# hjmkt/wrenc

Measured on AMD Instinct MI355X. Metric: all-intra encode fps at fixed QP (CTU RD search + final pass); bit-exactness vs the CPU oracle is checked in `parity`, higher is better.
Workload: dtype u8/i16/i32 (+i64 trellis costs, f32 RD cost)

## Files before the change

wrenc_amd/csrc/dev_common.h:

```cpp
#pragma once
#include <cstddef>
#include <type_traits>

namespace wrenc {

enum { PLANAR = 0, DC = 1, LT_CCLM = 81, L_CCLM = 82, T_CCLM = 83 };
enum { TREE_SINGLE = 0, TREE_DUAL_LUMA = 1, TREE_DUAL_CHROMA = 2 };

struct DevConst {
    int32_t W, H, qp, max_depth, ctu_cols, ctu_rows;
    int32_t lsc;
    uint32_t div_magic;
    uint32_t div_shift;
    int64_t lambda_q;
    float lambda_rd;
    float lambda_rd_chroma;
    int64_t ldq[1024];
    int64_t lv[1024];
    int64_t hb_luma[2][4][67];
    int64_t hb_chroma[4];
    int16_t dct[4][32][32];
    int16_t dct_t[4][32][32];
    uint8_t diag4[16][2];
    uint8_t diag_sb[4][64][2];
// ... 129 lines not shown
    UF<float> cur_cost;
    uint32_t pad3_;
    UF<float> cost;
    EvalPartsU e_best;
};

template <class T>
struct SF {
    T v;
    UF<T>* p;
    __device__ __forceinline__ T get() const { return v; }
    __device__ __forceinline__ operator T() const { return v; }
    __device__ __forceinline__ SF& operator=(T x) {
        v = x;
        p->set(x);
        return *this;
    }
    __device__ __forceinline__ SF& operator=(const SF& o) { return *this = o.v; }
    __device__ __forceinline__ SF& operator+=(int x) { return *this = (T)(v + x); }
    __device__ __forceinline__ SF& operator-=(int x) { return *this = (T)(v - x); }
};
struct EvalPartsSF {
    SF<uint32_t> ssd_y, ssd_c;
    SF<long long> lvl_y, lvl_c;
    __device__ __forceinline__ EvalParts get() const {
        EvalParts e;
        e.ssd_y = ssd_y;
        e.ssd_c = ssd_c;
        e.lvl_y = lvl_y;
        e.lvl_c = lvl_c;
        return e;
    }
};
struct LeafSF {
    SF<uint8_t> cont, op_ml, op_mc, op_act, bx, by, lg, need_refs0, need_refs1, need_org, cur_mode, mode,
        cclm_mode, holder, evalr, luma_mode, chroma_mode, best_cls, need_save, tile_best, slot;
    SF<float> best_cost, cur_cost, cost;
    EvalPartsSF e_best;
};
static_assert(sizeof(LeafSt) == 64, "snap_leaf reads the struct as 16 dwords");
__device__ __forceinline__ LeafSF snap_leaf(LeafSt& l) {
    __builtin_amdgcn_fence(__ATOMIC_ACQ_REL, "wavefront");
    const int w = ((const int*)&l)[LANE & 15];
    LeafSF s;
#define SNAP_U8(f)                                                                                          \
    s.f.v = (uint8_t)((unsigned)__builtin_amdgcn_readlane(w, (int)(offsetof(LeafSt, f) >> 2)) >> (8 * (offsetof(LeafSt, f) & 3))); \
    s.f.p = &l.f
#define SNAP_F32(f)                                                                       \
    s.f.v = __int_as_float(__builtin_amdgcn_readlane(w, (int)(offsetof(LeafSt, f) >> 2))); \
    s.f.p = &l.f
    SNAP_U8(cont); SNAP_U8(op_ml); SNAP_U8(op_mc); SNAP_U8(op_act); SNAP_U8(bx); SNAP_U8(by); SNAP_U8(lg);
    SNAP_U8(need_refs0); SNAP_U8(need_refs1); SNAP_U8(need_org); SNAP_U8(cur_mode); SNAP_U8(mode);
    SNAP_U8(cclm_mode); SNAP_U8(holder); SNAP_U8(evalr); SNAP_U8(luma_mode); SNAP_U8(chroma_mode);
    SNAP_U8(best_cls); SNAP_U8(need_save); SNAP_U8(tile_best); SNAP_U8(slot);
    SNAP_F32(best_cost); SNAP_F32(cur_cost); SNAP_F32(cost);
#undef SNAP_U8
#undef SNAP_F32
    constexpr int eb = (int)(offsetof(LeafSt, e_best) >> 2);
    s.e_best.ssd_y.v = (uint32_t)__builtin_amdgcn_readlane(w, eb + (int)(offsetof(EvalPartsU, ssd_y) >> 2));
    s.e_best.ssd_y.p = &l.e_best.ssd_y;
    s.e_best.ssd_c.v = (uint32_t)__builtin_amdgcn_readlane(w, eb + (int)(offsetof(EvalPartsU, ssd_c) >> 2));
    s.e_best.ssd_c.p = &l.e_best.ssd_c;
    {
        constexpr int o = eb + (int)(offsetof(EvalPartsU, lvl_y) >> 2);
        s.e_best.lvl_y.v = (long long)(((unsigned long long)(unsigned)__builtin_amdgcn_readlane(w, o + 1) << 32) |
                                       (unsigned)__builtin_amdgcn_readlane(w, o));
        s.e_best.lvl_y.p = &l.e_best.lvl_y;
    }
    {
        constexpr int o = eb + (int)(offsetof(EvalPartsU, lvl_c) >> 2);
        s.e_best.lvl_c.v = (long long)(((unsigned long long)(unsigned)__builtin_amdgcn_readlane(w, o + 1) << 32) |
                                       (unsigned)__builtin_amdgcn_readlane(w, o));
        s.e_best.lvl_c.p = &l.e_best.lvl_c;
    }
    return s;
}

struct CtuSt {
    UF<uint8_t> cont, in_leaf, xpar;
    UF<uint8_t> level, bx, by, lg, max_depth;
    uint8_t pad0_;
    UF<uint8_t> z, rl, rc;
    UF<uint8_t> rbx, rby, rlg;
    UF<uint8_t> ns_luma_cur, ns_chroma_cur;
    UF<uint8_t> pend, pbx, pby, plg, pslot;
    UF<uint8_t> dp0, dp1;
    UF<uint8_t> lvmode, lv_i, zend;
    UF<uint8_t> fz_on;
    UF<float> ret, ns_cost_cur;
    uint32_t pad1_;
    UF<float> ctu_cost;
    UF<float> lv_acc0, lv_acc1;
    LeafSt leaf;
};

struct XRes {
    uint32_t ssd_y, ssd_c;
    long long lvl_y, lvl_c;
};

constexpr int R_L0 = 0, R_A0 = 66, R_LF = 130, R_AF = 196, R_LC0 = 260, R_LC1 = 294, R_AC0 = 328, R_AC1 = 360;

typedef uint8_t ref_t;
struct __attribute__((aligned(16))) Lds {
    int16_t r1[1024];
    int32_t r2[512];
    ref_t refs[392];
    uint8_t recYtop[72];
    uint8_t recY[32 * 36];
    uint8_t recCtop[2][40];
    uint8_t recC[2][16 * 20];
    uint32_t decw[128];
    int32_t slot_xfer;
    uint32_t fsum;
    uint16_t q_pm[3][4][4];
    uint8_t cu_log2[64];
    uint8_t luma_mode[64];
    uint8_t chroma_mode[16];
    uint8_t left_mode[8];
    union {
        float ns_cost[4];
        uint32_t lev_was[4];
    };
    union {
        float split_cost[4];
        uint32_t lev_now[4];
    };
    uint8_t ns_luma[4], ns_chroma[4], child[4];
    CtuSt st;
    XRes xr[2];
};

struct Ctx {
    const CONST_AS DevConst* k;
    const GLOBAL_AS uint8_t* org;
    int W, WH;
    uint8_t* pred_scratch;
    GLOBAL_AS uint8_t* slots;
    unsigned long long* mismatch;
    int ctu_x, ctu_y;
    int cu32_mode;
    int write;
    int member;
    int store;
    int solo;
    int trace;
};

#ifndef WRENC_WPB
#define WRENC_WPB 4
#endif
constexpr int WPB = WRENC_WPB;
constexpr int kWorkgroupsPerCU = 20 / WPB;
constexpr int kTeam = 4;
struct LvBox {
    float ns_cost[3], split[3];
    uint8_t ml[3], mc[3];
    uint16_t pad_;
    uint32_t cnt[3][2];
    uint32_t srv_ready, job_posted, job_done, job_ack, job_fin;
    uint32_t job4_posted, job4_done, job4_ack, job4_fin;
    uint8_t job_bx, job_by, job4_bx, job4_by;
};
struct LdsTab {
    int32_t ldq[256];
    int32_t lv[256];
    int8_t fc[32][4];
    LvBox lvb;
#ifdef WRENC_EXP_LDS_PAD
    char pad[WRENC_EXP_LDS_PAD];
#endif
};
// ... 201 lines not shown
```

wrenc_amd/csrc/dev_search.h:

```cpp
#pragma once

namespace wrenc {

enum { K_SADLIST = 0, K_FULL = 1, K_NOP = 2, K_SADSEARCH = 3, K_CCLMSEARCH = 4, K_SERVE8 = 5, K_LEAF8 = 7, K_LEAF16 = 8, K_SPLIT8 = 9, K_SERVE4 = 10 };
enum { COPY_NONE = 0, COPY_SAVE = 1, COPY_RESTORE = 2, COPY_PULL = 3 };

#if defined(WRENC_TRACE) || defined(WRENC_EXHAUSTIVE_SPLITS)
constexpr bool kSplitCut = false;
#else
constexpr bool kSplitCut = true;
#endif

#if defined(WRENC_TRACE) || defined(WRENC_EXHAUSTIVE_CANDIDATES)
constexpr bool kCandidateCut = false;
#else
constexpr bool kCandidateCut = true;
#endif

struct Req {
    int kind;
    int comps;
    int tx, ty, tlg;
    int ml, mc;
    bool active;
    bool refs0, refs1;
    bool final;
    int stage;
    int copy_from;
    bool xchg;
    int tree;
    int pre_copy, copy_comps, copy_slot, copy_tx, copy_ty, copy_tlg;
    float fcur;
};

struct Res {
    uint32_t ssd_y, ssd_c;
    long long lvl_y, lvl_c;
    float v0;
    float vmin;
    int imin;
    int imin2;
};
__device__ __forceinline__ Res res_none() {
    Res r;
    r.ssd_y = 0;
    r.ssd_c = 0;
    r.lvl_y = 0;
    r.lvl_c = 0;
    r.v0 = r.vmin = 3.40282347e+38f;
    r.imin = 0;
    r.imin2 = 0;
    return r;
}

__device__ __forceinline__ float uni_f(float v) { return __int_as_float(uni(__float_as_int(v))); }

__device__ __forceinline__ unsigned checksum_weight(int i) { return (2u * (unsigned)i + 1u) * 0x9E3779B1u; }
__device__ __forceinline__ unsigned tile_checksum(int comp, int cx, int cy, int lg) {
    const int n = 1 << lg, nn = n * n, nb = comp ? 2 : 1;
    unsigned h = 0;
    for (int i = LANE; i < nb * nn; i += 64) {
        const int blk = i >> (2 * lg), ii = i & (nn - 1);
        h += (unsigned)rec_get(comp + blk, cx + (ii & (n - 1)), cy + (ii >> lg)) * checksum_weight(i);
    }
    return (unsigned)wave_sum_i32((int)h);
}

__device__ __forceinline__ void full_front(const Ctx& c, const Req& q, int comp, int mode, int rbase,
                                           CclmPick pick = CclmPick{}) {
    const int cs = comp ? 1 : 0;
    const int nb = comp ? 2 : 1;
    const int lg = q.tlg - cs;
    PROF_MARK(tr0_);
    if ((comp ? q.refs1 : q.refs0) && mode < LT_CCLM) build_refs(c, comp, q.tx, q.ty, q.tlg);
    if (q.final) {
        const unsigned h = tile_checksum(comp, q.tx >> cs, q.ty >> cs, lg);
        if (LANE == 0) SH.fsum = h;
        WSYNC();
    }
    PROF_MARK(t0_);
    PROF_ADD2(PH_REFS, tr0_, t0_);
    predict<true>(c, comp, q.tx, q.ty, q.tlg, mode, rbase, PRED_TILE, 0, pick);
    PROF_MARK(t1_);
    PROF_ADD2(PH_PREDICT, t0_, t1_);
    fwd_dct_lg(c, lg, nb, rbase);
    PROF_MARK(t2_);
    PROF_ADD2(PH_FDCT, t1_, t2_);
// ... 137 lines not shown
        int e0 = kNoMode, e1 = kNoMode, e2 = kNoMode, e3 = kNoMode, e4 = kNoMode, e5 = kNoMode;
        const int st = r == 1 ? 2 : 1;
        if (r == 0) {
            n = 13;
            lo = 2ULL | (7ULL << 8) | (13ULL << 16) | (18ULL << 24) | (23ULL << 32) | (29ULL << 40) | (34ULL << 48) | (39ULL << 56);
            hi = 45ULL | (50ULL << 8) | (55ULL << 16) | (60ULL << 24) | (66ULL << 32);
        } else if (six) {
            e0 = !(cm < 4) ? cm - 2 : kNoMode;
            e1 = !(cm + 2 > 66) ? cm + 2 : kNoMode;
            e2 = !(cm < 5) ? cm - 3 : kNoMode;
            e3 = !(cm < 3) ? cm - 1 : kNoMode;
            e4 = !(cm + 1 > 66) ? cm + 1 : kNoMode;
            e5 = !(cm + 3 > 66) ? cm + 3 : kNoMode;
            n = 6;
            lo = (unsigned long long)e0 | ((unsigned long long)e1 << 8) | ((unsigned long long)e2 << 16) | ((unsigned long long)e3 << 24) |
                 ((unsigned long long)e4 << 32) | ((unsigned long long)e5 << 40);
        } else {
            e0 = !(cm < 2 + st) ? cm - st : kNoMode;
            e1 = !(cm + st > 66) ? cm + st : kNoMode;
            n = 2;
            lo = (unsigned long long)e0 | ((unsigned long long)e1 << 8);
        }
        const unsigned acc = sad_list_angular(c, q.comps, q.tx, q.ty, q.tlg, n, lo, hi);
        const int my_mode = LANE < n ? (int)(((LANE < 8 ? lo : hi) >> (8 * (LANE & 7))) & 255u) : kNoMode;
        const unsigned s0 = (unsigned)__builtin_amdgcn_readlane((int)acc, 0), s1 = (unsigned)__builtin_amdgcn_readlane((int)acc, 1);
        bool traced = my_mode != kNoMode;
        if (r == 0) {
            const int key = my_mode != kNoMode ? (int)((acc << 4) | (unsigned)LANE) : 0x7FFFFFFF;
            const int kmin = wave_min_i32(key);
            const int j = (kmin & 15) + 2;
            cm = j < 8 ? (int)((0x3A5C90D0E08080ULL >> (7 * j)) & 127) : (int)((0x109E3764B53A2ULL >> (7 * (j - 8))) & 127);
            cur = (unsigned)kmin >> 4;
        } else if (six) {
            const unsigned s2 = (unsigned)__builtin_amdgcn_readlane((int)acc, 2), s3 = (unsigned)__builtin_amdgcn_readlane((int)acc, 3);
            const unsigned s4 = (unsigned)__builtin_amdgcn_readlane((int)acc, 4), s5 = (unsigned)__builtin_amdgcn_readlane((int)acc, 5);
            const unsigned c0 = e0 != kNoMode ? s0 : kNoSad, c1 = e1 != kNoMode ? s1 : kNoSad;
            const unsigned mn = min(min(cur, c0), c1);
            int d = 0;
            if (cur == mn) {
            } else if (c0 == mn) {
                d = -2;
                cur = c0;
            } else {
                d = 2;
                cur = c1;
            }
            const int elo = d < 0 ? e2 : (d == 0 ? e3 : e4), ehi = d < 0 ? e3 : (d == 0 ? e4 : e5);
            const unsigned slo = d < 0 ? s2 : (d == 0 ? s3 : s4), shi = d < 0 ? s3 : (d == 0 ? s4 : s5);
            const unsigned p0 = elo != kNoMode ? slo : kNoSad, p1 = ehi != kNoMode ? shi : kNoSad;
            cm += d;
            const unsigned mn2 = min(min(cur, p0), p1);
            if (cur == mn2) {
            } else if (p0 == mn2) {
                cm -= 1;
                cur = p0;
            } else {
                cm += 1;
                cur = p1;
            }
            const int ilo = d < 0 ? 2 : (d == 0 ? 3 : 4);
            traced = traced && (LANE < 2 || LANE == ilo || LANE == ilo + 1);
        } else {
            const unsigned c0 = e0 != kNoMode ? s0 : kNoSad, c1 = e1 != kNoMode ? s1 : kNoSad;
            const unsigned mn = min(min(cur, c0), c1);
            if (cur == mn) {
            } else if (c0 == mn) {
                cm -= st;
                cur = c0;
            } else {
                cm += st;
                cur = c1;
            }
        }
        if (c.trace && traced)
            TRACE_REC(c.ctu_x + q.tx, c.ctu_y + q.ty, q.tlg, q.tree, (q.comps & 1) ? 0 : 2, (q.comps & 1) ? my_mode : 0, my_mode,
                      __float_as_int((float)acc));
    }
    cm_out = cm;
    smin_out = cur;
}

__device__ __forceinline__ Res leaf8_search(const Ctx& c, const Req& q, int* overflow);
__device__ __forceinline__ Res leaf16_search(const Ctx& c, const Req& q, int* overflow);
__device__ __forceinline__ Res split8_search(const Ctx& c, const Req& q, int* overflow);
__device__ __forceinline__ void serve_pack4(const Ctx& c, const Req& q, int* overflow);
__device__ __forceinline__ void serve_pack8(const Ctx& c, const Req& q, int* overflow);

__device__ __forceinline__ int cclm_probe(const Ctx& c, int tx, int ty, int lg, int tree, CclmParams* all) {
    const int lane = lane_fresh();
    const unsigned acc = sad_list_cclm(c, tx, ty, lg, all);
    const unsigned lt = (unsigned)__builtin_amdgcn_readlane((int)acc, 0), t = (unsigned)__builtin_amdgcn_readlane((int)acc, 1),
                   l = (unsigned)__builtin_amdgcn_readlane((int)acc, 2);
    if (c.trace && lane < 3)
        TRACE_REC(c.ctu_x + tx, c.ctu_y + ty, lg, tree, 2, 0, lane == 0 ? LT_CCLM : (lane == 1 ? T_CCLM : L_CCLM),
                  __float_as_int((float)acc));
    return (lt <= t && lt <= l) ? LT_CCLM : (t <= l ? T_CCLM : L_CCLM);
}

__device__ __forceinline__ int cclm_pred4_lane(const Ctx& c, const Req& q, const CclmPick& pick, int pl, int x, int y) {
    int v = 128;
    if (!pick.flat128) {
        const int ds = cclm_ds6(c, q.tx, q.ty, 2 * y, 2 * x, pick.avail_l);
        v = (M24(ds, pl ? pick.a1 : pick.a0) >> (pl ? pick.k1 : pick.k0)) + (pl ? pick.b1 : pick.b0);
        v = min(max(v, 0), 255);
    }
    return v;
}

template <bool TEAM, bool D3>
__device__ __forceinline__ Res evaluate(const Ctx& c, const PicBufs& pb, const Req& q, int* overflow) {
    Res r = res_none();
    PROF_MARK(tcp0_);
    if (q.pre_copy != COPY_NONE)
        copy_block(c, q.pre_copy, q.copy_comps, q.copy_slot, q.copy_tx, q.copy_ty, q.copy_tlg, q.copy_from);
    PROF_MARK(tcp1_);
    PROF_ADD2(PH_COPY, tcp0_, tcp1_);
    if (q.kind == K_NOP) return r;
    if (q.stage) stage_org_leaf(c, q.stage, q.tx, q.ty, q.tlg);
    if (q.kind == K_LEAF8) return leaf8_search(c, q, overflow);
    if (q.kind == K_LEAF16) return leaf16_search(c, q, overflow);
    if (D3 && q.kind == K_SPLIT8) return split8_search(c, q, overflow);
    if (TEAM && q.kind == K_SERVE8) {
        serve_pack8(c, q, overflow);
        return r;
    }
    if (TEAM && D3 && q.kind == K_SERVE4) {
        serve_pack4(c, q, overflow);
        return r;
    }
    int mc = q.mc;
    CclmPick cpick_ = CclmPick{};
    if (q.kind == K_CCLMSEARCH) {
        if (q.tlg > 4) stage_org(c, 2, q.tx, q.ty, q.tlg);
        CclmParams call_;
        mc = cclm_probe(c, q.tx, q.ty, q.tlg, q.tree, &call_);
        r.imin = mc;
        cpick_ = cclm_pick(call_, 2 * cclm_mode_index(mc));
    }
    if (q.kind == K_FULL || q.kind == K_CCLMSEARCH) {
#pragma unroll 1
        for (int round = 0; round < 2; ++round) {
            const int cset = q.comps & (1 << round);
            if (!cset) continue;
            if (q.active) {
#pragma unroll 1
                for (int comp = 0; comp < 2; ++comp)
                    if ((cset >> comp) & 1) {
                        PROF_MARK(tf0_);
                        full_front(c, q, comp, comp ? mc : q.ml, 0, cpick_);
                        PROF_MARK(tf1_);
                        PROF_ADD2(PH_PSZ + ((q.tlg - 2) * 2 + comp), tf0_, tf1_);
                        PROF_ADD2(PH_PCNT + ((q.tlg - 2) * 2 + comp), 0, 1);
                    }
            }
            PROF_MARK(ts0_);
            bool any_y = false, any_c = false;
            {
                bool any = false;
                long long lvl = 0;
                if (q.active)
                    lvl = quantize_solo(c, q.tlg - round, round ? 2 : 1, overflow, &any);
                if (round) {
                    r.lvl_c = lvl;
                    any_c = any;
                } else {
                    r.lvl_y = lvl;
                    any_y = any;
                }
            }
            PROF_MARK(ts1_);
            PROF_ADD2(PH_QZ + ((q.tlg - 2) & 3), ts0_, ts1_);
            if (!q.active) {
                PROF_ADD2(PH_SKIP, ts0_, ts1_);
                continue;
            }
#pragma unroll 1
            for (int comp = 0; comp < 2; ++comp) {
                if (!((cset >> comp) & 1)) continue;
                PROF_MARK(tb0_);
                const uint32_t ssd = full_back(c, pb, q, comp, 0, comp ? any_c : any_y);
                PROF_MARK(tb1_);
                PROF_ADD2(PH_PSZ + ((q.tlg - 2) * 2 + comp), tb0_, tb1_);
                if (comp)
                    r.ssd_c = ssd;
                else
                    r.ssd_y = ssd;
            }
        }
        return r;
    }
    PROF_MARK(tr0_);
    if (q.refs0 && (q.comps & 1)) build_refs(c, 0, q.tx, q.ty, q.tlg);
    if (q.refs1 && (q.comps & 2)) build_refs(c, 1, q.tx, q.ty, q.tlg);
    if (q.tlg > 4) stage_org(c, q.comps, q.tx, q.ty, q.tlg);
    PROF_MARK(t0_);
    PROF_ADD2(PH_REFS, tr0_, t0_);
    if (q.kind == K_SADSEARCH) {
        constexpr unsigned kNoSad = 0xFFFFFFFFu;
        int cm;
        unsigned smin = kNoSad;
        sad_search(c, q, cm, smin);
        r.imin = uni(cm);
        r.vmin = smin == kNoSad ? 3.40282347e+38f : uni_f((float)smin);
    } else {
// ... 767 lines not shown
}

__device__ __forceinline__ Res leaf16_search(const Ctx& c, const Req& q, int* overflow) {
    Res r = res_none();
    const int lane = lane_fresh();
    if (q.refs0) build_refs(c, 0, q.tx, q.ty, 4);
    if (q.refs1) build_refs(c, 1, q.tx, q.ty, 4);
    LeafBest best = leaf_best_init(PLANAR);
    const MpmList mpl_ = mpm_list(c, q.tx, q.ty, 4);
    {
        PROF_MARK(la0_);
        const Pack16Out a = pack16_eval(c, q, 2, PLANAR, DC, overflow);
        leaf_candidate(c, q.tx, q.ty, 4, TREE_SINGLE, mpl_, best, 0, PLANAR, pack_parts(a, 0));
        leaf_candidate(c, q.tx, q.ty, 4, TREE_SINGLE, mpl_, best, 1, DC, pack_parts(a, 1));
        pack16_to_tile(c, q, 2, best.win);
        PROF_MARK(la1_);
        PROF_ADD2(PH_LEAF + 4, la0_, la1_);
    }
    int cm;
    unsigned smin;
    PROF_MARK(ls0_);
    sad_search(c, q, cm, smin);
    PROF_MARK(ls1_);
    PROF_ADD2(PH_LEAF + 5, ls0_, ls1_);
    cm = uni(cm);
    const int lo = !(cm < 3) ? cm - 1 : kNoMode, hi = !(cm + 1 > 66) ? cm + 1 : kNoMode;
    {
        const Pack16Out b = pack16_eval(c, q, 2, cm, lo, overflow);
        best.win = -1;
        leaf_candidate(c, q.tx, q.ty, 4, TREE_SINGLE, mpl_, best, 0, cm, pack_parts(b, 0));
        if (lo != kNoMode) leaf_candidate(c, q.tx, q.ty, 4, TREE_SINGLE, mpl_, best, 1, lo, pack_parts(b, 1));
        if (best.win >= 0) pack16_to_tile(c, q, 2, best.win);
    }
    PROF_MARK(lb1_);
    PROF_ADD2(PH_LEAF + 6, ls1_, lb1_);
    if (hi != kNoMode) {
        const Pack16Out b = pack16_eval(c, q, 1, hi, kNoMode, overflow);
        best.win = -1;
        leaf_candidate(c, q.tx, q.ty, 4, TREE_SINGLE, mpl_, best, 0, hi, pack_parts(b, 0));
        if (best.win >= 0) pack16_to_tile(c, q, 1, best.win);
    }
    PROF_MARK(lc1_);
    PROF_ADD2(PH_LEAF + 7, lb1_, lc1_);
    r.vmin = best.cost;
    r.imin = best.mode;
    r.imin2 = best.mode;
    r.ssd_y = best.e.ssd_y;
    r.ssd_c = best.e.ssd_c;
    r.lvl_y = best.e.lvl_y;
    r.lvl_c = best.e.lvl_c;
    return r;
}

__device__ __forceinline__ void fill_maps(int bx, int by, int lg, int luma_mode, int chroma_mode, bool luma,
                                          bool chroma) {
    const int l4 = lg - 2;
    if (luma && LANE < (1 << (2 * l4))) {
        const int idx = ((by >> 2) + (LANE >> l4)) * 8 + (bx >> 2) + (LANE & ((1 << l4) - 1));
        SH.cu_log2[idx] = (uint8_t)lg;
        SH.luma_mode[idx] = (uint8_t)luma_mode;
    }
    if (chroma) {
        const int l8 = max(l4 - 1, 0);
        if (LANE < (1 << (2 * l8)))
            SH.chroma_mode[((by >> 3) + (LANE >> l8)) * 4 + (bx >> 3) + (LANE & ((1 << l8) - 1))] = (uint8_t)chroma_mode;
    }
    WSYNC();
}


__device__ __forceinline__ bool split_floor_cut(const Ctx& c, float partial, int n, int fi, bool chroma, float unsplit,
                                                float* bound) {
    if (!kSplitCut) return false;
    float b = partial;
    const float f = c.k->split_floor[fi];
    for (int i = 0; i < n; ++i) b = b + f;
    if (chroma) b = b + c.k->split_floor[1];
    b = uni_f(b);
    if (!(b > unsplit)) return false;
    *bound = b;
    return true;
}

__device__ __forceinline__ Res split8_search(const Ctx& c, const Req& q, int* overflow) {
    Res r = res_none();
    float split8 = 0.0f;
#pragma unroll 1
    for (int i8 = 0; i8 < 4; ++i8) {
        Req ql = {};
        ql.comps = 1;
        ql.tx = q.tx + (i8 & 1) * 4;
        ql.ty = q.ty + (i8 >> 1) * 4;
        ql.tlg = 2;
        ql.refs0 = true;
        ql.refs1 = false;
        ql.tree = TREE_DUAL_LUMA;
        if (split_floor_cut(c, split8, 4 - i8, 0, true, q.fcur, &r.vmin)) {
            PROF_ADD2(PH_CUT + 0, 0, 4 - i8);
            PROF_ADD2(PH_CUT + 1, 0, 1);
            PROF_ADD2(PH_CUT + 4, 0, split8 > q.fcur ? 0 : 1);
            return r;
        }
        PROF_MARK(l4g0_);
        stage_org_leaf(c, 1, ql.tx, ql.ty, 2);
        PROF_MARK(l4g1_);
        PROF_ADD2(PH_L4 + 0, l4g0_, l4g1_);
        const Res rl = leaf4_search(c, ql, overflow);
        fill_maps(ql.tx, ql.ty, 2, rl.imin, 0, true, false);
        split8 = uni_f(split8 + rl.vmin);
    }
    if (split_floor_cut(c, split8, 0, 0, true, q.fcur, &r.vmin)) {
        PROF_ADD2(PH_CUT + 1, 0, 1);
        PROF_ADD2(PH_CUT + 4, 0, split8 > q.fcur ? 0 : 1);
        return r;
    }
    Req qc = {};
    qc.tx = q.tx;
    qc.ty = q.ty;
    qc.comps = 2;
    qc.tlg = 3;
    qc.ml = 0;
    qc.mc = uni((int)SH.luma_mode[((q.ty + 4) >> 2) * 8 + ((q.tx + 4) >> 2)]);
    qc.refs0 = false;
    qc.refs1 = true;
    qc.tree = TREE_DUAL_CHROMA;
    PROF_MARK(l4c0_);
    stage_org_leaf(c, 2, q.tx, q.ty, 3);
    const Res rc = leafc4_search(c, qc, overflow);
    fill_maps(q.tx, q.ty, 3, 0, rc.imin, false, true);
    PROF_MARK(l4c1_);
    PROF_ADD2(PH_L4 + 4, l4c0_, l4c1_);
    r.vmin = uni_f(split8 + rc.vmin);
    return r;
}

__device__ __forceinline__ void req_full(Req& q, int comps, int tx, int ty, int tlg, int ml, int mc, bool active,
                                         bool refs0, bool refs1, bool final) {
    q.kind = K_FULL;
    q.comps = comps;
    q.tx = tx;
    q.ty = ty;
    q.tlg = tlg;
    q.ml = ml;
    q.mc = mc;
    q.active = active;
    q.refs0 = refs0;
    q.refs1 = refs1;
    q.final = final;
    q.stage = (final && tlg <= 4) ? comps : 0;
    q.pre_copy = COPY_NONE;
    q.xchg = false;
}

__device__ __forceinline__ void req_copy(Req& q, int mode, int comps, int slot, int tx, int ty, int tlg) {
    q.pre_copy = mode;
    q.copy_comps = comps;
    q.copy_slot = slot;
    q.copy_tx = tx;
    q.copy_ty = ty;
    q.copy_tlg = tlg;
    q.copy_from = -1;
}

enum {
    C_START = 0, C_PLANAR = 1, C_DCM = 2, C_LIST = 3, C_F0 = 6, C_F1 = 7, C_F2 = 8, C_CCLM = 11, C_DM = 12,
    C_L8 = 20, C_L16 = 21, C_WINNER = 22
};

__device__ __forceinline__ void leaf_init(LeafSt& s, int bx, int by, int lg, int slot = 0) {
    s.cont = C_START;
    s.bx = (uint8_t)bx;
    s.by = (uint8_t)by;
    s.lg = (uint8_t)lg;
    s.need_refs0 = 1;
    s.need_refs1 = 1;
    s.need_org = lg <= 4 ? 1 : 0;
    s.need_save = 0;
    s.tile_best = 0;
    s.slot = (uint8_t)slot;
}

__device__ __forceinline__ void leaf_attach_save(LeafSF& s, Req& q) {
    q.pre_copy = COPY_NONE;
    if (s.need_save) {
        req_copy(q, COPY_SAVE, 3, s.slot, s.bx, s.by, s.lg);
// ... 428 lines not shown
        by = (i >> 1) * 16;
    } else {
        const int qd = i >> 2, sb = i & 3;
        bx = (qd & 1) * 16 + (sb & 1) * 8;
        by = (qd >> 1) * 16 + (sb >> 1) * 8;
    }
}
__device__ __forceinline__ void lv_pull_maps(const Ctx& c, int from, int bx, int by, int lg) {
    const Lds& src = team_lds(c, from);
    const int l4 = lg - 2;
    if (LANE < (1 << (2 * l4))) {
        const int idx = ((by >> 2) + (LANE >> l4)) * 8 + (bx >> 2) + (LANE & ((1 << l4) - 1));
        SH.cu_log2[idx] = src.cu_log2[idx];
        SH.luma_mode[idx] = src.luma_mode[idx];
    }
    const int l8 = lg - 3;
    if (LANE < (1 << (2 * l8))) {
        const int idx = ((by >> 3) + (LANE >> l8)) * 4 + (bx >> 3) + (LANE & ((1 << l8) - 1));
        SH.chroma_mode[idx] = src.chroma_mode[idx];
    }
    WSYNC();
}
__device__ __forceinline__ void lv_pull(const Ctx& c, int from, int tx, int ty, int tlg) {
    const Lds& src = team_lds(c, from);
    const int words = 1 << (2 * tlg - 2);
    for (int w = LANE; w < words; w += 64) {
        const int row = (4 * w) >> tlg, col = (4 * w) & ((1 << tlg) - 1);
        const int at = (ty + row) * 36 + tx + col + 4;
        *(uint32_t*)&SH.recY[at] = *(const uint32_t*)&src.recY[at];
    }
    const int lg = tlg - 1;
    const int cwords = 1 << (2 * lg - 2);
    for (int w = LANE; w < 2 * cwords; w += 64) {
        const int pl = w >= cwords ? 1 : 0;
        const int ww = w - pl * cwords;
        const int row = (4 * ww) >> lg, col = (4 * ww) & ((1 << lg) - 1);
        const int at = ((ty >> 1) + row) * 20 + (tx >> 1) + col + 4;
        *(uint32_t*)&SH.recC[pl][at] = *(const uint32_t*)&src.recC[pl][at];
    }
    WSYNC();
}
__device__ __forceinline__ float lv_decide(const Ctx& c, int L, int idx) {
    const int me = c.member;
    const int dl = c.k->max_depth;
    const int nmem = L == 0 ? kTeam : dl - L + 1;
    PROF_MARK(tx0_);
    lv_meet(L, 0, (idx + 1) * nmem);
    PROF_MARK(tx1_);
    PROF_ADD2(PH_XCHG, tx0_, tx1_);
    PROF_ADDM(2, tx0_, tx1_);
    const float ns = uni_f(SHT.lvb.ns_cost[L]), sp = uni_f(SHT.lvb.split[L]);
    const int ml = uni((int)SHT.lvb.ml[L]), mc = uni((int)SHT.lvb.mc[L]);
    int bx, by;
    lv_node(L, idx, bx, by);
    const int lg = 5 - L;
    const bool unsplit = sp > ns;
    if (unsplit) {
        if (me > L) lv_pull(c, L, bx, by, lg);
        fill_maps(bx, by, lg, ml, mc, true, true);
    } else if (me == L || me > dl) {
        lv_pull(c, L + 1, bx, by, lg);
        lv_pull_maps(c, L + 1, bx, by, lg);
    }
    PROF_MARK(tx2_);
    lv_meet(L, 1, (idx + 1) * nmem);
    PROF_MARK(tx3_);
    PROF_ADD2(PH_COPY, tx1_, tx2_);
    PROF_ADD2(PH_XCHG, tx2_, tx3_);
    PROF_ADDM(2, tx2_, tx3_);
    return unsplit ? ns : sp;
}
__device__ __forceinline__ void lv_post_unsplit(int L, float ns, int ml, int mc) {
    if (LANE == 0) {
        SHT.lvb.ns_cost[L] = ns;
        SHT.lvb.ml[L] = (uint8_t)ml;
        SHT.lvb.mc[L] = (uint8_t)mc;
    }
}
__device__ __forceinline__ void lv_post_split(int L, float sp) {
    if (LANE == 0) SHT.lvb.split[L] = sp;
}


enum { T_START = 0, T_ENTER = 1, T_NODE_LEAF = 2, T_REGEN_DONE = 6, T_RETURN = 7, T_FINAL_Z = 8, T_FZ_TAIL = 9, T_FZ_NEXT = 10,
       T_LV_UNIT = 11, T_LV_LEAFDONE = 12, T_LV_UP = 13, T_SPLIT8 = 14, T_LV_SERVE = 15 };

template <bool TEAM, bool D3>
__device__ __forceinline__ bool ctu_step(Ctx& c, const Res& r, Req& q) {
    CtuSt& t = SH.st;
    bool in_leaf = t.in_leaf != 0;
    int cont = t.cont;
    for (;;) {
        if (in_leaf) {
            LeafSF ls = snap_leaf(t.leaf);
            if ((TEAM && !t.lvmode) ? leaf_step_team(c, t, ls, q, t.xpar ^ 1, r) : leaf_step(c, ls, r, q)) {
                if (t.pend) {
                    req_copy(q, COPY_SAVE, t.pend, t.pslot, t.pbx, t.pby, t.plg);
                    t.pend = 0;
                }
                t.cont = (uint8_t)cont;
                t.in_leaf = 1;
                return true;
            }
            t.in_leaf = 0;
            in_leaf = false;
        }
        switch (cont) {
        case T_START:
            t.level = 0;
            t.bx = 0;
            t.by = 0;
            cont = T_ENTER;
            break;
        case T_ENTER: {
            const int lg = 5 - t.level;
            t.lg = (uint8_t)lg;
            leaf_init(t.leaf, t.bx, t.by, lg, (!TEAM && t.level < t.max_depth) ? 1 + t.level : 0);
            if (TEAM && !t.lvmode) t.leaf.cont = TC_START;
            in_leaf = true;
            cont = T_NODE_LEAF;
            break;
        }
        case T_NODE_LEAF: {
            const float ns = t.leaf.cost;
            const int ml = t.leaf.luma_mode, mc = t.leaf.chroma_mode;
            const int level = t.level, lg = t.lg;
            t.ns_cost_cur = ns;
            t.ns_luma_cur = (uint8_t)ml;
            t.ns_chroma_cur = (uint8_t)mc;
            fill_maps(t.bx, t.by, lg, ml, mc, true, true);
            if (level == 0) c.cu32_mode = ml;
            if (t.max_depth - level == 0) {
                t.ret = ns;
                cont = T_RETURN;
                break;
            }
            if (TEAM) {
                if (t.dp0) {
                    const int dp = t.dp0, dq = t.dp1;
                    t.dp0 = 0;
                    copy_block(c, COPY_PULL, (dp >> 1) & 3, 0, (dq & 7) << 2, (dq >> 3) << 2, (dp >> 5) + 2, (dp >> 3) & 3);
                }
                t.lvmode = 1;
                t.lv_i = 0;
                t.lv_acc0 = 0.0f;
                t.lv_acc1 = 0.0f;
                if (c.member == 0) lv_post_unsplit(0, ns, ml, mc);
                cont = (c.member == 0 || c.member > t.max_depth) ? T_LV_UP : T_LV_UNIT;
                break;
            }
            t.pend = (uint8_t)(lg == 3 ? 3 : (mc >= LT_CCLM ? 2 : 0));
            t.pbx = t.bx;
            t.pby = t.by;
            t.plg = (uint8_t)lg;
            t.pslot = (uint8_t)(1 + level);
            if (LANE == 0) {
                SH.ns_cost[level] = ns;
                SH.ns_luma[level] = (uint8_t)ml;
                SH.ns_chroma[level] = (uint8_t)mc;
                SH.split_cost[level] = 0.0f;
                SH.child[level] = 0;
            }
            WSYNC();
            if (lg > 3 || !D3) {
                float bound;
                if (split_floor_cut(c, 0.0f, 4, 2 + level + 1, false, ns, &bound)) {
                    PROF_ADD2(PH_CUT + 2 + level, 0, 4);
                    PROF_ADD2(PH_CUT + 5, 0, 1);
                    t.pend = 0;
                    t.ret = ns;
                    cont = T_RETURN;
                    break;
                }
                t.level = (uint8_t)(level + 1);
                cont = T_ENTER;
                break;
            }
            req_full(q, 3, t.bx, t.by, 3, 0, 0, true, false, false, false);
            q.kind = K_SPLIT8;
            q.stage = 0;
            q.tree = TREE_DUAL_LUMA;
            q.fcur = ns;
            if (t.pend) {
                req_copy(q, COPY_SAVE, t.pend, t.pslot, t.pbx, t.pby, t.plg);
                t.pend = 0;
            }
            t.cont = T_SPLIT8;
            return true;
        }
        case T_SPLIT8: {
            if constexpr (D3) {
                const float split8 = r.vmin;
                if (TEAM && t.lvmode) {
                    lv_post_split(2, split8);
                    cont = T_LV_UP;
                    break;
                }
                if (split8 > t.ns_cost_cur) {
                    t.rbx = t.bx;
                    t.rby = t.by;
                    t.rlg = t.lg;
                    t.rl = t.ns_luma_cur;
                    t.rc = t.ns_chroma_cur;
                    q.kind = K_NOP;
                    q.xchg = false;
                    req_copy(q, COPY_RESTORE, 3, 1 + t.level, t.rbx, t.rby, t.rlg);
                    t.cont = T_REGEN_DONE;
                    return true;
                }
                t.ret = split8;
                cont = T_RETURN;
                break;
            }
            }
            break;
        case T_REGEN_DONE:
            fill_maps(t.rbx, t.rby, t.rlg, t.rl, t.rc, true, true);
            t.ret = uni_f(SH.ns_cost[t.level]);
            cont = T_RETURN;
            break;
        case T_RETURN: {
            const int level = t.level;
            if (level == 0) {
                t.ctu_cost = t.ret;
                t.z = 0;
                if (TEAM && t.dp0) {
                    q.kind = K_NOP;
                    q.pre_copy = COPY_NONE;
                    q.xchg = false;
                    t.cont = T_RETURN;
                    return true;
                }
                t.z = (uint8_t)(TEAM ? 16 * c.member : 0);
                t.zend = (uint8_t)(TEAM ? 16 * c.member + 16 : 64);
                cont = T_FINAL_Z;
                break;
            }
            const int pl = level - 1;
            const int psz = 1 << (5 - pl);
            const int pbx = t.bx & ~(psz - 1), pby = t.by & ~(psz - 1);
            const float acc = uni_f(uni_f(SH.split_cost[pl]) + t.ret);
            const int ch = uni((int)SH.child[pl]) + 1;
            WSYNC();
            if (LANE == 0) {
                SH.split_cost[pl] = acc;
                SH.child[pl] = (uint8_t)ch;
            }
            WSYNC();
            const float ns_p = uni_f(SH.ns_cost[pl]);
            float bound;
            const bool lost = ch < 4 ? split_floor_cut(c, acc, 4 - ch, 2 + level, false, ns_p, &bound) : acc > ns_p;
            if (ch < 4 && !lost) {
                t.bx = (uint8_t)(pbx + (ch & 1) * (psz >> 1));
                t.by = (uint8_t)(pby + (ch >> 1) * (psz >> 1));
                cont = T_ENTER;
                break;
            }
            PROF_ADD2(PH_CUT + 1 + level, 0, 4 - ch);
            PROF_ADD2(PH_CUT + 5, 0, (ch < 4 && !(acc > ns_p)) ? 1 : 0);
            t.bx = (uint8_t)pbx;
            t.by = (uint8_t)pby;
            t.level = (uint8_t)pl;
            if (lost) {
                t.rbx = (uint8_t)pbx;
                t.rby = (uint8_t)pby;
                t.rlg = (uint8_t)(5 - pl);
                t.rl = (uint8_t)uni((int)SH.ns_luma[pl]);
                t.rc = (uint8_t)uni((int)SH.ns_chroma[pl]);
                q.kind = K_NOP;
                q.xchg = false;
                req_copy(q, COPY_RESTORE, 3, 1 + pl, t.rbx, t.rby, t.rlg);
                t.cont = T_REGEN_DONE;
                return true;
            }
            t.ret = acc;
            break;
        }
        case T_LV_UNIT: {
            if constexpr (TEAM) {
                const int me = c.member, i = t.lv_i;
                int bx, by;
                lv_node(me == 1 ? 1 : 2, i, bx, by);
                t.bx = (uint8_t)bx;
                t.by = (uint8_t)by;
                if constexpr (D3) {
                    if (me == 3) {
                        t.lg = 3;
                        req_full(q, 3, bx, by, 3, 0, 0, true, false, false, false);
                        q.kind = K_SPLIT8;
                        q.stage = 0;
                        q.tree = TREE_DUAL_LUMA;
                        q.fcur = __builtin_inff();
                        t.cont = T_SPLIT8;
                        return true;
// ... 343 lines not shown
```

Baseline: 225.9.

## Fuse 8x8 node unsplit and split search into one node8 request

New measurement: 230.0 (median of 6 runs). 1.8% higher.

```diff
diff --git a/wrenc_amd/csrc/dev_common.h b/wrenc_amd/csrc/dev_common.h
--- a/wrenc_amd/csrc/dev_common.h
+++ b/wrenc_amd/csrc/dev_common.h
@@ -235,12 +235,13 @@
     uint8_t pad0_;
     UF<uint8_t> z, rl, rc;
     UF<uint8_t> rbx, rby, rlg;
-    UF<uint8_t> ns_luma_cur, ns_chroma_cur;
+    uint8_t pad2_[2];
     UF<uint8_t> pend, pbx, pby, plg, pslot;
     UF<uint8_t> dp0, dp1;
     UF<uint8_t> lvmode, lv_i, zend;
     UF<uint8_t> fz_on;
-    UF<float> ret, ns_cost_cur;
+    UF<float> ret;
+    uint32_t pad3_;
     uint32_t pad1_;
     UF<float> ctu_cost;
     UF<float> lv_acc0, lv_acc1;
diff --git a/wrenc_amd/csrc/dev_search.h b/wrenc_amd/csrc/dev_search.h
--- a/wrenc_amd/csrc/dev_search.h
+++ b/wrenc_amd/csrc/dev_search.h
@@ -2,7 +2,8 @@
 
 namespace wrenc {
 
-enum { K_SADLIST = 0, K_FULL = 1, K_NOP = 2, K_SADSEARCH = 3, K_CCLMSEARCH = 4, K_SERVE8 = 5, K_LEAF8 = 7, K_LEAF16 = 8, K_SPLIT8 = 9, K_SERVE4 = 10 };
+enum { K_SADLIST = 0, K_FULL = 1, K_NOP = 2, K_SADSEARCH = 3, K_CCLMSEARCH = 4, K_SERVE8 = 5, K_LEAF8 = 7, K_LEAF16 = 8, K_SPLIT8 = 9, K_SERVE4 = 10,
+       K_NODE8 = 11 };
 enum { COPY_NONE = 0, COPY_SAVE = 1, COPY_RESTORE = 2, COPY_PULL = 3 };
 
 #if defined(WRENC_TRACE) || defined(WRENC_EXHAUSTIVE_SPLITS)
@@ -306,7 +307,8 @@
 
 __device__ __forceinline__ Res leaf8_search(const Ctx& c, const Req& q, int* overflow);
 __device__ __forceinline__ Res leaf16_search(const Ctx& c, const Req& q, int* overflow);
-__device__ __forceinline__ Res split8_search(const Ctx& c, const Req& q, int* overflow);
+__device__ __forceinline__ Res split8_search(const Ctx& c, const Req& q, int* overflow, int* leaves = nullptr);
+__device__ __forceinline__ void fill_maps(int bx, int by, int lg, int luma_mode, int chroma_mode, bool luma, bool chroma);
 __device__ __forceinline__ void serve_pack4(const Ctx& c, const Req& q, int* overflow);
 __device__ __forceinline__ void serve_pack8(const Ctx& c, const Req& q, int* overflow);
 
@@ -329,6 +331,39 @@
         v = min(max(v, 0), 255);
     }
     return v;
+}
+
+__device__ __forceinline__ float node8_search(const Ctx& c, int tx, int ty, int* overflow) {
+    Req qn = {};
+    qn.comps = 3;
+    qn.tx = tx;
+    qn.ty = ty;
+    qn.tlg = 3;
+    qn.refs0 = true;
+    qn.refs1 = true;
+    qn.tree = TREE_SINGLE;
+    stage_org_leaf(c, 3, tx, ty, 3);
+    const Res ru = leaf8_search(c, qn, overflow);
+    const float ns = ru.vmin;
+    const int ml = ru.imin, mc = ru.imin2;
+    fill_maps(tx, ty, 3, ml, mc, true, true);
+    unsigned kept;
+    {
+        const int lane = lane_fresh();
+        kept = (unsigned)rec_get(0, tx + (lane & 7), ty + (lane >> 3));
+        if (lane < 32) kept |= (unsigned)rec_get(1 + (lane >> 4), (tx >> 1) + (lane & 3), (ty >> 1) + ((lane & 15) >> 2)) << 8;
+    }
+    qn.fcur = ns;
+    int leaves = 0;
+    const float split8 = split8_search(c, qn, overflow, &leaves).vmin;
+    if (!(split8 > ns)) return split8;
+    if (leaves) {
+        const int lane = lane_fresh();
+        rec_put(0, tx + (lane & 7), ty + (lane >> 3), (int)(kept & 255u));
+        if (lane < 32) rec_put(1 + (lane >> 4), (tx >> 1) + (lane & 3), (ty >> 1) + ((lane & 15) >> 2), (int)(kept >> 8));
+        fill_maps(tx, ty, 3, ml, mc, true, true);
+    }
+    return ns;
 }
 
 template <bool TEAM, bool D3>
@@ -341,9 +376,14 @@
     PROF_ADD2(PH_COPY, tcp0_, tcp1_);
     if (q.kind == K_NOP) return r;
     if (q.stage) stage_org_leaf(c, q.stage, q.tx, q.ty, q.tlg);
-    if (q.kind == K_LEAF8) return leaf8_search(c, q, overflow);
+    constexpr bool kNodes = !TEAM && D3;
+    if (kNodes && q.kind == K_NODE8) {
+        r.vmin = node8_search(c, q.tx, q.ty, overflow);
+        return r;
+    }
+    if (!kNodes && q.kind == K_LEAF8) return leaf8_search(c, q, overflow);
     if (q.kind == K_LEAF16) return leaf16_search(c, q, overflow);
-    if (D3 && q.kind == K_SPLIT8) return split8_search(c, q, overflow);
+    if (TEAM && D3 && q.kind == K_SPLIT8) return split8_search(c, q, overflow);
     if (TEAM && q.kind == K_SERVE8) {
         serve_pack8(c, q, overflow);
         return r;
@@ -1277,7 +1317,7 @@
     return true;
 }
 
-__device__ __forceinline__ Res split8_search(const Ctx& c, const Req& q, int* overflow) {
+__device__ __forceinline__ Res split8_search(const Ctx& c, const Req& q, int* overflow, int* leaves) {
     Res r = res_none();
     float split8 = 0.0f;
 #pragma unroll 1
@@ -1296,6 +1336,7 @@
             PROF_ADD2(PH_CUT + 4, 0, split8 > q.fcur ? 0 : 1);
             return r;
         }
+        if (leaves) *leaves = 1;
         PROF_MARK(l4g0_);
         stage_org_leaf(c, 1, ql.tx, ql.ty, 2);
         PROF_MARK(l4g1_);
@@ -1890,7 +1931,7 @@
 }
 
 
-enum { T_START = 0, T_ENTER = 1, T_NODE_LEAF = 2, T_REGEN_DONE = 6, T_RETURN = 7, T_FINAL_Z = 8, T_FZ_TAIL = 9, T_FZ_NEXT = 10,
+enum { T_START = 0, T_ENTER = 1, T_NODE_LEAF = 2, T_NODE8 = 3, T_REGEN_DONE = 6, T_RETURN = 7, T_FINAL_Z = 8, T_FZ_TAIL = 9, T_FZ_NEXT = 10,
        T_LV_UNIT = 11, T_LV_LEAFDONE = 12, T_LV_UP = 13, T_SPLIT8 = 14, T_LV_SERVE = 15 };
 
 template <bool TEAM, bool D3>
@@ -1923,6 +1964,17 @@
         case T_ENTER: {
             const int lg = 5 - t.level;
             t.lg = (uint8_t)lg;
+            if (!TEAM && D3 && lg == 3) {
+                req_full(q, 3, t.bx, t.by, 3, 0, 0, true, false, false, false);
+                q.kind = K_NODE8;
+                q.tree = TREE_SINGLE;
+                if (t.pend) {
+                    req_copy(q, COPY_SAVE, t.pend, t.pslot, t.pbx, t.pby, t.plg);
+                    t.pend = 0;
+                }
+                t.cont = T_NODE8;
+                return true;
+            }
             leaf_init(t.leaf, t.bx, t.by, lg, (!TEAM && t.level < t.max_depth) ? 1 + t.level : 0);
             if (TEAM && !t.lvmode) t.leaf.cont = TC_START;
             in_leaf = true;
@@ -1933,9 +1985,6 @@
             const float ns = t.leaf.cost;
             const int ml = t.leaf.luma_mode, mc = t.leaf.chroma_mode;
             const int level = t.level, lg = t.lg;
-            t.ns_cost_cur = ns;
-            t.ns_luma_cur = (uint8_t)ml;
-            t.ns_chroma_cur = (uint8_t)mc;
             fill_maps(t.bx, t.by, lg, ml, mc, true, true);
             if (level == 0) c.cu32_mode = ml;
             if (t.max_depth - level == 0) {
@@ -1957,7 +2006,7 @@
                 cont = (c.member == 0 || c.member > t.max_depth) ? T_LV_UP : T_LV_UNIT;
                 break;
             }
-            t.pend = (uint8_t)(lg == 3 ? 3 : (mc >= LT_CCLM ? 2 : 0));
+            t.pend = (uint8_t)(mc >= LT_CCLM ? 2 : 0);
             t.pbx = t.bx;
             t.pby = t.by;
             t.plg = (uint8_t)lg;
@@ -1970,54 +2019,31 @@
                 SH.child[level] = 0;
             }
             WSYNC();
-            if (lg > 3 || !D3) {
-                float bound;
-                if (split_floor_cut(c, 0.0f, 4, 2 + level + 1, false, ns, &bound)) {
-                    PROF_ADD2(PH_CUT + 2 + level, 0, 4);
-                    PROF_ADD2(PH_CUT + 5, 0, 1);
-                    t.pend = 0;
-                    t.ret = ns;
-                    cont = T_RETURN;
-                    break;
-                }
-                t.level = (uint8_t)(level + 1);
-                cont = T_ENTER;
+            float bound;
+            if (split_floor_cut(c, 0.0f, 4, 2 + level + 1, false, ns, &bound)) {
+                PROF_ADD2(PH_CUT + 2 + level, 0, 4);
+                PROF_ADD2(PH_CUT + 5, 0, 1);
+                t.pend = 0;
+                t.ret = ns;
+                cont = T_RETURN;
                 break;
             }
-            req_full(q, 3, t.bx, t.by, 3, 0, 0, true, false, false, false);
-            q.kind = K_SPLIT8;
-            q.stage = 0;
-            q.tree = TREE_DUAL_LUMA;
-            q.fcur = ns;
-            if (t.pend) {
-                req_copy(q, COPY_SAVE, t.pend, t.pslot, t.pbx, t.pby, t.plg);
-                t.pend = 0;
-            }
-            t.cont = T_SPLIT8;
-            return true;
-        }
+            t.level = (uint8_t)(level + 1);
+            cont = T_ENTER;
+            break;
+        }
+        case T_NODE8: {
+            if constexpr (!TEAM && D3) {
+                t.ret = r.vmin;
+                cont = T_RETURN;
+                break;
+            }
+            }
+            break;
         case T_SPLIT8: {
-            if constexpr (D3) {
-                const float split8 = r.vmin;
-                if (TEAM && t.lvmode) {
-                    lv_post_split(2, split8);
-                    cont = T_LV_UP;
-                    break;
-                }
-                if (split8 > t.ns_cost_cur) {
-                    t.rbx = t.bx;
-                    t.rby = t.by;
-                    t.rlg = t.lg;
-                    t.rl = t.ns_luma_cur;
-                    t.rc = t.ns_chroma_cur;
-                    q.kind = K_NOP;
-                    q.xchg = false;
-                    req_copy(q, COPY_RESTORE, 3, 1 + t.level, t.rbx, t.rby, t.rlg);
-                    t.cont = T_REGEN_DONE;
-                    return true;
-                }
-                t.ret = split8;
-                cont = T_RETURN;
+            if constexpr (TEAM && D3) {
+                lv_post_split(2, r.vmin);
+                cont = T_LV_UP;
                 break;
             }
             }
```
